# SJTU-IPADS/cocytus

Hardware: AMD Instinct MI355X
Metric: GiB/s device-resident RS(3,2) encode+decode, 4 KiB values (higher is better)
Workload: dtype u8

## Files before the change

cocytus_amd/csrc/cec_kernels.hpp:

```cpp
#pragma once

#include <hip/hip_runtime.h>
#include <stdint.h>

#include "gf256.hpp"

namespace cec {

constexpr int kTile = 4096;
constexpr int kBlock = 256;
constexpr int kBlockLog2 = 8;
constexpr uint64_t kLineBytes = 128;
static_assert(kBlock == 1 << kBlockLog2, "kBlock must be a power of two");
constexpr int kMaxStreams = 48;
constexpr int kPatN = 16;
constexpr int kPatL = 4;

enum : int32_t { kModeWrite = 0, kModeXor = 1 };

struct alignas(16) Pattern {
    int32_t n_in;
    int32_t n_out;
    int32_t in_stream[kPatN];
    int32_t in_src[kPatN];
// ... 283 lines not shown
                if (i < n_in) x[i] = ld16(in[i], pos);
#pragma unroll
            for (int l = 0; l < LT; ++l) {
                acc[l] = make_uint4(0, 0, 0, 0);
                if (l < n_out && is_acc(l)) acc[l] = ld16(out[l], pos);
            }
        } else {
#pragma unroll
            for (int i = 0; i < NT; ++i)
                if (i < n_in) x[i] = gather16(in[i], pos, cnt);
#pragma unroll
            for (int l = 0; l < LT; ++l) {
                acc[l] = make_uint4(0, 0, 0, 0);
                if (l < n_out && is_acc(l)) acc[l] = gather16(out[l], pos, cnt);
            }
        }
        if constexpr (Eng::kStaged) {
            const uint32_t nb = static_cast<uint32_t>(P->lds_rows) * 256u;
            if (nb) {
                const uint4 *src = reinterpret_cast<const uint4 *>(a.rows) + P->lds_row_base * 16;
                for (uint32_t b = threadIdx.x; b < nb / 16; b += blockDim.x) cec_lds_rows[b] = src[b];
                __syncthreads();
            }
            if (!active) continue;
        }
        compute_chunk<NT, LT, Eng>(P, n_in, n_out, x, acc, lds);
        if (wide) {
            bool wt = false;
            if constexpr (!Eng::kStaged) {
                wt = (a.flags & kFlagWriteThrough) != 0;
                if constexpr (S > kNarrowStreams) wt = wt || g >= a.wt_from;
            }
            if (wt) {
#pragma unroll
                for (int l = 0; l < LT; ++l)
                    if (l < n_out) st16_wt(out[l], pos, acc[l]);
            } else {
#pragma unroll
                for (int l = 0; l < LT; ++l)
                    if (l < n_out) st16(out[l], pos, acc[l]);
            }
        } else {
#pragma unroll
            for (int l = 0; l < LT; ++l)
                if (l < n_out) scatter16(out[l], pos, cnt, acc[l]);
        }
    }
    if constexpr (kSysRel) {
        __builtin_amdgcn_fence(__ATOMIC_RELEASE, "");
        __asm__ volatile("s_waitcnt vmcnt(0)" ::: "memory");
    }
}

constexpr int kScrubStreams = 24;

struct ScrubArgs {
    const uint8_t *base[kScrubStreams];
    const Tile *tiles;
    const Pattern *pattern;
    uint32_t *words;
    uint32_t *counter;
    uint64_t implicit_len;
    uint32_t n_tiles;
    uint32_t split_shift;
    uint32_t grid;
    uint32_t syn_shift;
};

template <int NT, int LT, bool kExact>
__global__ __launch_bounds__(kBlock) void scrub_kernel(ScrubArgs a) {
    const uint32_t sh = a.split_shift;
    const uint32_t g = blockIdx.x;
    if (g >= a.grid) return;
    const uint32_t t = g >> sh;
    const uint32_t part = g & ((1u << sh) - 1u);
    const uint32_t lane = (part << (kBlockLog2 - sh)) + threadIdx.x;
    const TileRef tr = load_tile(a, t);
    const CEC_CONST Pattern *P = as_const(a.pattern);
    const int n_in = kExact ? NT : P->n_in;
    const int n_out = kExact ? LT : P->n_out;

    const uint8_t *in[NT];
    const uint8_t *par[LT];
    uint64_t mis = 0;
#pragma unroll
    for (int i = 0; i < NT; ++i) {
        in[i] = nullptr;
        if (i < n_in) {
            in[i] = a.base[i] + tr.off;
            mis |= reinterpret_cast<uint64_t>(in[i]);
        }
    }
#pragma unroll
    for (int l = 0; l < LT; ++l) {
        par[l] = nullptr;
        if (l < n_out) {
            par[l] = a.base[n_in + l] + tr.off;
            mis |= reinterpret_cast<uint64_t>(par[l]);
        }
    }

    const uint32_t pos = lane * 16;
    if (pos >= tr.len) return;
    const uint32_t cnt = min(16u, tr.len - pos);
    uint4 x[NT];
    uint4 acc[LT];
// ... 317 lines not shown
```

cocytus_amd/csrc/cec_runtime.hip:

```cpp
#include <hip/hip_runtime.h>

#include <algorithm>
#include <atomic>
#include <chrono>
#include <cerrno>
#include <cstdarg>
#include <cstdio>
#include <cstdlib>
#include <cstring>
#include <map>
#include <mutex>
#include <string>
#include <vector>

#include "../../include/cocytus_ec.h"
#include "../../include/galois.h"
#include "../../include/jerasure.h"
#include "../../include/reed_sol.h"
#include "cec_hostplan.hpp"
#include "cec_kernels.hpp"
#include "cec_poolbook.hpp"
#include "gf256.hpp"

#define CEC_API extern "C" __attribute__((visibility("default")))
// ... 112 lines not shown

template <int NT, int LT, class Eng, int kAcc, bool kExact, int S = kMaxStreams, bool kSysRel = false>
static void launch_k(const CombineArgsN<S> &a, int grid, size_t lds, hipStream_t s) {
    hipLaunchKernelGGL((combine_kernel<NT, LT, Eng, kAcc, kExact, S, kSysRel>), dim3(grid),
                       dim3(kBlock >> a.split_shift), lds, s, a);
}

static CombineArgsN<kNarrowStreams> narrow_args(const CombineArgs &w) {
    CombineArgsN<kNarrowStreams> a;
    memset(&a, 0, sizeof a);
    for (int i = 0; i < kNarrowStreams; ++i) a.base[i] = w.base[i];
    a.tiles = w.tiles;
    a.patterns = w.patterns;
    a.rows = w.rows;
    a.implicit_len = w.implicit_len;
    a.n_tiles = w.n_tiles;
    a.split_shift = w.split_shift;
    a.grid = w.grid;
    a.flags = w.flags;
    return a;
}

template <class Eng>
static bool launch_narrow(int acc, const CombineArgsN<kNarrowStreams> &a, int grid, size_t lds, hipStream_t s) {
    const bool rel = (a.flags & kFlagSysRelease) != 0;
    if (acc == kAccAll && rel) launch_k<1, 1, Eng, kAccAll, true, kNarrowStreams, true>(a, grid, lds, s);
    else if (acc == kAccAll) launch_k<1, 1, Eng, kAccAll, true, kNarrowStreams>(a, grid, lds, s);
    else if (acc == kAccNone && rel) launch_k<1, 1, Eng, kAccNone, true, kNarrowStreams, true>(a, grid, lds, s);
    else if (acc == kAccNone) launch_k<1, 1, Eng, kAccNone, true, kNarrowStreams>(a, grid, lds, s);
    else return false;
    return true;
}

#define CEC_EXACT_WRITES(X, N) X(N, 1, kAccNone) X(N, 2, kAccNone) X(N, 3, kAccNone) X(N, 4, kAccNone)
#define CEC_EXACT_SHAPES(X)                                                                      \
    CEC_EXACT_WRITES(X, 1) CEC_EXACT_WRITES(X, 2) CEC_EXACT_WRITES(X, 3) CEC_EXACT_WRITES(X, 4)  \
    CEC_EXACT_WRITES(X, 5) CEC_EXACT_WRITES(X, 6) CEC_EXACT_WRITES(X, 7) CEC_EXACT_WRITES(X, 8)  \
    X(1, 1, kAccAll) X(2, 1, kAccAll) X(2, 2, kAccAll) X(2, 3, kAccAll) X(2, 4, kAccAll)         \
    X(2, 2, kAccAllButLast) X(2, 3, kAccAllButLast) X(2, 4, kAccAllButLast)

template <class Eng>
static bool launch_exact(int n, int l, int acc, const CombineArgs &a, int grid, size_t lds,
                         hipStream_t s) {
#define CEC_X(N, L, A)                                           \
    if (n == N && l == L && acc == A) {                          \
        launch_k<N, L, Eng, A, true>(a, grid, lds, s);       \
        return true;                                             \
    }
    CEC_EXACT_SHAPES(CEC_X)
#undef CEC_X
    return false;
}

static bool has_exact(int n, int l, int acc) {
#define CEC_X(N, L, A) if (n == N && l == L && acc == A) return true;
    CEC_EXACT_SHAPES(CEC_X)
#undef CEC_X
    return false;
}

struct Capacity {
    int nt, lt;
};
#define CEC_LT_RUNGS(lt, NT, K)                  \
    if (lt <= 1) { K(NT, 1) }                    \
    else if (lt <= 2) { K(NT, 2) }               \
    else { K(NT, 4) }
#define CEC_CAPACITY_RUNGS_FROM_4(nt, lt, K)     \
    if (nt <= 4) { CEC_LT_RUNGS(lt, 4, K) }      \
    else if (nt <= 8) { CEC_LT_RUNGS(lt, 8, K) } \
    else { CEC_LT_RUNGS(lt, 16, K) }
#define CEC_CAPACITY_RUNGS(nt, lt, K)            \
    if (nt <= 2) { CEC_LT_RUNGS(lt, 2, K) }      \
    else { CEC_CAPACITY_RUNGS_FROM_4(nt, lt, K) }

template <class Eng>
static Capacity launch_generic(int nt, int lt, const CombineArgs &a, int grid, size_t lds, hipStream_t s) {
#define CEC_G(NT, LT)                                              \
    launch_k<NT, LT, Eng, kAccRuntime, false>(a, grid, lds, s);   \
    return {NT, LT};
    CEC_CAPACITY_RUNGS(nt, lt, CEC_G)
#undef CEC_G
}

static bool exact_shape(const std::vector<Pattern> &pats, const std::vector<char> *used, int *n, int *l,
                        int *acc) {
    const Pattern *p0 = nullptr;
    for (size_t i = 0; i < pats.size(); ++i) {
        if (used && !(*used)[i]) continue;
        const Pattern &p = pats[i];
        if (!p0) {
            p0 = &p;
            continue;
        }
        if (p.n_in != p0->n_in || p.n_out != p0->n_out) return false;
        for (int o = 0; o < p.n_out; ++o)
            if (p.out_mode[o] != p0->out_mode[o]) return false;
    }
    if (!p0) return false;
    int nx = 0;
    for (int o = 0; o < p0->n_out; ++o) nx += p0->out_mode[o] == kModeXor;
    if (nx == 0) *acc = kAccNone;
    else if (nx == p0->n_out) *acc = kAccAll;
    else if (nx == p0->n_out - 1 && p0->out_mode[p0->n_out - 1] == kModeWrite) *acc = kAccAllButLast;
    else return false;
    *n = p0->n_in;
    *l = p0->n_out;
    return true;
}

#include "cec_combo.inc"

static inline size_t tiles_of(uint64_t off, uint32_t len) {
    return len ? static_cast<size_t>((off % kTile + len + kTile - 1) / kTile) : 0;
}
static inline size_t append_tiles(Tile *t, uint64_t off, uint64_t src_off, uint32_t len,
                                  uint32_t pattern) {
    size_t n = 0;
    for (uint32_t o = 0; o < len;) {
        const uint32_t phase = static_cast<uint32_t>((off + o) % kTile);
        const uint32_t step = std::min<uint32_t>(kTile - phase, len - o);
        t[n++] = Tile{off + o, src_off + o, step, pattern};
        o += step;
    }
    return n;
}
static inline int64_t count_line_tiles(const Tile *t, size_t n) {
    int64_t c = 0;
    for (size_t i = 0; i < n; ++i) c += t[i].len == kTile && (t[i].off & (kLineBytes - 1)) == 0;
    return c;
}

struct cec_plan {
    int device = -1;
    int n_ext = 0;
    int64_t n_tiles = 0;
    uint64_t total = 0;
    bool overlap = false;
    int64_t n_line_tiles = 0;
    Tile *d_tiles = nullptr;
    uint32_t max_pattern = 0;
    uint64_t max_end = 0;
    int max_end_ext = -1;
    std::vector<Tile> h_tiles;
    mutable Tracker uses;
};

CEC_API int cec_plan_destroy(cec_plan *p) {
    if (!p) return CEC_OK;
    int rc = CEC_OK;
    if (hipError_t e = p->uses.wait(p->device); e != hipSuccess)
        rc = fail(CEC_EHIP, "cec_plan_destroy: a launch of this plan failed: %s", hipGetErrorString(e));
    dev_cache().release(p->device, p->d_tiles, sizeof(Tile) * p->n_tiles);
    delete p;
    return rc;
}

CEC_API int cec_plan_release_stream(cec_plan *p, void *stream) {
    if (!p) return fail(CEC_EINVAL, "cec_plan_release_stream: plan is NULL");
    if (hipError_t e = p->uses.release(p->device, static_cast<hipStream_t>(stream)); e != hipSuccess)
        return fail(CEC_EHIP, "cec_plan_release_stream: %s", hipGetErrorString(e));
    return CEC_OK;
}
CEC_API int cec_plan_tracked_streams(const cec_plan *p) { return p ? static_cast<int>(p->uses.size()) : 0; }

CEC_API int cec_plan_create(cec_plan **out, const cec_extent *ext, int n, void *stream) {
    if (!out || n < 0 || (n > 0 && !ext)) return fail(CEC_EINVAL, "cec_plan_create: bad args");
    *out = nullptr;
    int dev;
    if (int r = current_device(&dev)) return r;
    cec_plan *p = new (std::nothrow) cec_plan;
    if (!p) return fail(CEC_ENOMEM, "cec_plan_create: host allocation");
    p->device = dev;
    p->n_ext = n;
    for (int e = 0; e < n; ++e) {
        p->max_pattern = std::max(p->max_pattern, ext[e].pattern);
        if (!ext[e].len) continue;
        const uint64_t end = ext[e].off > UINT64_MAX - ext[e].len ? UINT64_MAX : ext[e].off + ext[e].len;
        if (p->max_end_ext < 0 || end > p->max_end) {
            p->max_end = end;
            p->max_end_ext = e;
        }
    }
    size_t total_tiles = 0;
    for (int e = 0; e < n; ++e) total_tiles += tiles_of(ext[e].off, ext[e].len);
    p->h_tiles.resize(total_tiles);
    size_t nt = 0;
    for (int e = 0; e < n; ++e) {
        p->total += ext[e].len;
        nt += append_tiles(p->h_tiles.data() + nt, ext[e].off, ext[e].src_off, ext[e].len, ext[e].pattern);
    }
    if (p->h_tiles.size() > 0xFFFFFFFFull) {
        delete p;
        return fail(CEC_EINVAL, "cec_plan_create: more than 2^32 tiles");
    }
    p->n_tiles = static_cast<int64_t>(p->h_tiles.size());
    p->n_line_tiles = count_line_tiles(p->h_tiles.data(), p->h_tiles.size());
    {
        std::vector<std::pair<uint64_t, uint64_t>> r;
        r.reserve(n);
        for (int e = 0; e < n; ++e)
            if (ext[e].len) r.emplace_back(ext[e].off, ext[e].off + ext[e].len);
        std::sort(r.begin(), r.end());
        for (size_t i = 1; i < r.size(); ++i)
            if (r[i].first < r[i - 1].second) { p->overlap = true; break; }
    }
    hipStream_t s = static_cast<hipStream_t>(stream);
    if (p->n_tiles > 0) {
        const size_t bytes = sizeof(Tile) * p->n_tiles;
        p->d_tiles = static_cast<Tile *>(dev_cache().acquire(dev, bytes));
        if (!p->d_tiles) {
            delete p;
            return fail(CEC_ENOMEM, "cec_plan_create: %zu bytes of tiles", bytes);
        }
        if (hipMemcpyAsync(p->d_tiles, p->h_tiles.data(), bytes, hipMemcpyHostToDevice, s) != hipSuccess) {
            (void)hipGetLastError();
            cec_plan_destroy(p);
            return fail(CEC_EHIP, "cec_plan_create: tile upload failed");
        }
        p->uses.note(s);
    }
    *out = p;
    return CEC_OK;
}

CEC_API int cec_plan_num_extents(const cec_plan *p) { return p ? p->n_ext : 0; }
CEC_API int64_t cec_plan_num_tiles(const cec_plan *p) { return p ? p->n_tiles : 0; }
CEC_API uint64_t cec_plan_total_bytes(const cec_plan *p) { return p ? p->total : 0; }

struct TileSource {
    const Tile *tiles = nullptr;
    uint64_t n_tiles = 0;
    uint64_t n_line_tiles = 0;
    uint64_t implicit_len = 0;
    Tracker *uses = nullptr;

    static int of_plan(const cec_plan *plan, int dev, TileSource *out) {
        if (plan->device != dev)
            return fail(CEC_EINVAL, "plan built on device %d used on device %d", plan->device, dev);
        *out = {plan->d_tiles, static_cast<uint64_t>(plan->n_tiles), static_cast<uint64_t>(plan->n_line_tiles), 0,
                &plan->uses};
        return CEC_OK;
    }
    static int of_region(uint64_t len, TileSource *out) {
        const uint64_t n = (len + kTile - 1) / kTile;
        if (n > 0xFFFFFFFFull) return fail(CEC_EINVAL, "region too large");
        *out = {nullptr, n, n, len, nullptr};
        return CEC_OK;
    }
    static TileSource window(const Tile *d, const Tile *h, size_t n) {
        return {d, n, static_cast<uint64_t>(count_line_tiles(h, n)), 0, nullptr};
    }
    static TileSource whole_units(const Tile *d, size_t n) { return {d, n, n, 0, nullptr}; }
};

struct WaveTiles {
    Tile *h;
    size_t n = 0;
    std::vector<size_t> first;
    int cur = -1;
    explicit WaveTiles(Tile *host) : h(host) {}
    void begin_wave() { first.push_back(n); }
    void enter(int wave) {
        if (wave != cur) begin_wave();
        cur = wave;
    }
    void add(uint64_t off, uint64_t src_off, uint32_t len, uint32_t pattern) {
        n += append_tiles(h + n, off, src_off, len, pattern);
    }
    int waves() const { return static_cast<int>(first.size()); }
    TileSource all(const Tile *d) const { return TileSource::window(d, h, n); }
    TileSource window(int w, const Tile *d) const {
        const size_t lo = first[w], hi = w + 1 < waves() ? first[w + 1] : n;
        return TileSource::window(d + lo, h + lo, hi - lo);
    }
};

static uint32_t split_shift_for(const Streams &st, const TileSource &src) {
    static const int forced = [] {
        const char *e = getenv("CEC_SPLIT_SHIFT");
        return e && *e ? std::min(2, std::max(0, atoi(e))) : -1;
    }();
    if (forced >= 0) return static_cast<uint32_t>(forced);
    uintptr_t mis = 0;
    for (int i = 0; i < kMaxStreams; ++i) mis |= reinterpret_cast<uintptr_t>(st.base[i]);
    const bool full = src.n_line_tiles * 4 >= src.n_tiles * 3;
    return full && (mis & (kLineBytes - 1)) == 0 ? 2u : 0u;
}

static std::atomic<int> g_waves_per_cu{[] {
    const char *e = getenv("CEC_WAVES_PER_CU");
    return e && *e ? std::max(0, atoi(e)) : 0;
}()};
static int waves_per_cu_cap() { return g_waves_per_cu.load(std::memory_order_relaxed); }

static size_t occupancy_lds(int dev, uint32_t split_shift) {
    const int cap = waves_per_cu_cap();
    if (cap <= 0) return 0;
    const int waves_per_wg = (kBlock >> split_shift) / 64;
    const int wgs = std::max(1, cap / std::max(1, waves_per_wg));
    const size_t per_cu = g_dev[dev].lds_per_cu;
    const size_t lds = per_cu / static_cast<size_t>(wgs);
    return std::min<size_t>(65536, lds > 256 ? lds - 256 : 0);
}

enum { kStoreAuto = 0, kStoreNt = 1, kStoreWt = 2 };
// ... 3 lines not shown
    if (!strcmp(e, "wt")) return static_cast<int>(kStoreWt);
    if (!strcmp(e, "nt")) return static_cast<int>(kStoreNt);
    fprintf(stderr, "libcocytus_ec: CEC_STORE_POLICY=%s is not nt, wt or auto; using auto\n", e);
    return static_cast<int>(kStoreAuto);
}();
static uint64_t parse_byte_count(const char *name, uint64_t dflt) {
    const char *e = getenv(name);
    if (!e || !*e) return dflt;
    char *end = nullptr;
    errno = 0;
    const unsigned long long v = (*e >= '0' && *e <= '9') ? strtoull(e, &end, 0) : 0;
    if (!(*e >= '0' && *e <= '9') || !end || *end || errno == ERANGE) {
        fprintf(stderr, "libcocytus_ec: %s=%s is not a byte count; using %llu\n", name, e,
                static_cast<unsigned long long>(dflt));
        return dflt;
    }
    return static_cast<uint64_t>(v);
}
static const uint64_t g_wt_max_bytes = parse_byte_count("CEC_WT_MAX_BYTES", uint64_t(512) << 20);
CEC_API int cec_internal_store_policy(uint64_t *wt_max_bytes) {
    if (wt_max_bytes) *wt_max_bytes = g_wt_max_bytes;
    return g_store_policy;
}
static const uint64_t g_wt_tail_bytes = parse_byte_count("CEC_WT_TAIL_BYTES", uint64_t(96) << 20);

struct StoreChoice {
    bool all;
    uint64_t from;
};
static StoreChoice write_through(uint64_t n_tiles, uint32_t split_shift, int lt, uint64_t streamed) {
    if (g_store_policy != kStoreAuto) return {g_store_policy == kStoreWt, kNoWtTail};
    if (streamed <= g_wt_max_bytes) return {true, kNoWtTail};
    if (g_wt_tail_bytes == 0 || lt <= 0) return {false, kNoWtTail};
    const uint64_t per_item = static_cast<uint64_t>(lt) * (kTile >> split_shift);
    const uint64_t items = g_wt_tail_bytes / per_item + (g_wt_tail_bytes % per_item != 0);
    const uint64_t n_work = n_tiles << split_shift;
    if (items >= n_work) return {true, kNoWtTail};
    return {false, n_work - items};
}
CEC_API int cec_internal_wt_from(uint64_t n_tiles, uint32_t split_shift, int lt, uint64_t streamed,
                                 uint64_t *wt_tail_bytes, uint64_t *wt_from) {
    if (split_shift > 2 || n_tiles > 0xFFFFFFFFull) return fail(CEC_EINVAL, "cec_internal_wt_from: bad args");
    const StoreChoice c = write_through(n_tiles, split_shift, lt, streamed);
    if (wt_tail_bytes) *wt_tail_bytes = g_wt_tail_bytes;
    if (wt_from) *wt_from = c.from;
    return c.all ? 2 : c.from != kNoWtTail ? 1 : 0;
}

struct LaunchShape {
    int nt = 1, lt = 0, max_rows = 0;
    bool exact = false;
    int en = 0, el = 0, eacc = 0;
    int streams = 0;
};

static LaunchShape launch_shape(const std::vector<Pattern> &pats, const std::vector<char> *used) {
    LaunchShape sh;
    for (size_t i = 0; i < pats.size(); ++i) {
        if (used && !(*used)[i]) continue;
        sh.nt = std::max(sh.nt, pats[i].n_in);
        sh.lt = std::max(sh.lt, pats[i].n_out);
        sh.max_rows = std::max(sh.max_rows, pats[i].lds_rows);
        for (int j = 0; j < pats[i].n_in; ++j) sh.streams = std::max(sh.streams, pats[i].in_stream[j] + 1);
        for (int j = 0; j < pats[i].n_out; ++j) sh.streams = std::max(sh.streams, pats[i].out_stream[j] + 1);
    }
    sh.exact = exact_shape(pats, used, &sh.en, &sh.el, &sh.eacc);
    return sh;
}

enum KernelKind { kKindNarrow, kKindExact, kKindGeneric };
static_assert(kKindNarrow == CEC_KERNEL_NARROW && kKindExact == CEC_KERNEL_EXACT &&
                  kKindGeneric == CEC_KERNEL_GENERIC, "cec_launch_record::kind");
static_assert(kAccNone == CEC_ACC_NONE && kAccAll == CEC_ACC_ALL && kAccAllButLast == CEC_ACC_ALL_BUT_LAST &&
                  kAccRuntime == CEC_ACC_RUNTIME, "cec_launch_record::acc");
static_assert(kFlagSysRelease == CEC_LAUNCH_SYS_RELEASE && kFlagWriteThrough == CEC_LAUNCH_WRITE_THROUGH &&
                  kFlagWtTail == CEC_LAUNCH_WT_TAIL, "cec_launch_record::flags");

static thread_local cec_launch_record t_last_launch = {0, -1, 0, 0, -1, -1, 0, 0, 0, 0, 0, kNoWtTail};

static void record_launch(int kind, Capacity cap, int acc, bool lds, uint32_t split_shift, uint32_t flags,
                          uint32_t grid, uint64_t n_tiles, size_t lds_bytes, uint64_t wt_from = kNoWtTail) {
    t_last_launch = {t_last_launch.seq + 1, kind, cap.nt, cap.lt, acc, lds ? CEC_ENGINE_LDS : CEC_ENGINE_PERM,
                     split_shift, flags, grid, n_tiles, lds_bytes, wt_from};
}

CEC_API int cec_last_launch(cec_launch_record *out) {
    if (!out) return fail(CEC_EINVAL, "cec_last_launch: out is NULL");
    *out = t_last_launch;
    return CEC_OK;
}

static thread_local int t_fail_after = -1;
CEC_API int cec_internal_fail_launch(int after) {
    t_fail_after = after < 0 ? -1 : after;
    return CEC_OK;
}
static int launch_countdown() {
    if (t_fail_after == 0) {
        t_fail_after = -1;
        return fail(CEC_EHIP, "injected launch failure (cec_internal_fail_launch)");
    }
    if (t_fail_after > 0) --t_fail_after;
    return CEC_OK;
}

static int pattern_tables(int dev, const std::vector<Pattern> &pats, const std::vector<uint8_t> &rows,
                          hipStream_t s, PatEntry **entry) {
    std::string key(reinterpret_cast<const char *>(pats.data()), pats.size() * sizeof(Pattern));
    key.append(reinterpret_cast<const char *>(rows.data()), rows.size());
    return pattern_get(dev, std::move(key), s, entry);
}

struct Tables {
    const uint8_t *d;
    size_t n_pats;
    const Pattern *host;
    const std::vector<char> *used;
};

static bool stream_layout_ok(const uint8_t *const *bases, int slots, const Tables &tb) {
    for (size_t q = 0; q < tb.n_pats; ++q) {
        if (tb.used && (q >= tb.used->size() || !(*tb.used)[q])) continue;
        const Pattern &p = tb.host[q];
        for (int i = 0; i < p.n_in; ++i)
            if (p.in_stream[i] >= slots || !bases[p.in_stream[i]]) return false;
        for (int l = 0; l < p.n_out; ++l)
            if (p.out_stream[l] >= slots || !bases[p.out_stream[l]]) return false;
    }
    return true;
}

static bool layout_ok_for(const CombineArgs &a, const CombineArgsN<kNarrowStreams> *narrow, const Tables &tb) {
    return narrow ? stream_layout_ok(narrow->base, kNarrowStreams, tb) : stream_layout_ok(a.base, kMaxStreams, tb);
}

static int launch_combine(int dev, const Streams &st, const Tables &tb, const LaunchShape &sh, bool lds,
                          const TileSource &src, hipStream_t stream, uint32_t flags = 0, bool *released = nullptr) {
    if (st.refused) return fail(CEC_EINVAL, "internal: an op names more than %d byte streams; not launched", kMaxStreams);
    CombineArgs a;
    memset(&a, 0, sizeof a);
    a.flags = flags;
    const bool exact_k = sh.exact && has_exact(sh.en, sh.el, sh.eacc);
    const KernelKind kind =
        exact_k && sh.en == 1 && sh.el == 1 && sh.streams <= kNarrowStreams &&
                (sh.eacc == kAccAll || sh.eacc == kAccNone)
            ? kKindNarrow
            : exact_k ? kKindExact : kKindGeneric;
    for (int i = 0; i < kMaxStreams; ++i) a.base[i] = st.base[i];
    a.tiles = src.tiles;
    a.implicit_len = src.implicit_len;
    a.patterns = reinterpret_cast<const Pattern *>(tb.d);
    a.rows = tb.d + tb.n_pats * sizeof(Pattern);
    a.n_tiles = static_cast<uint32_t>(src.n_tiles);
    a.split_shift = split_shift_for(st, src);
    const StoreChoice wt = write_through(src.n_tiles, a.split_shift, sh.lt,
                                         src.n_tiles * kTile * static_cast<uint64_t>(sh.nt + sh.lt));
    a.wt_from = kind == kKindNarrow || lds ? kNoWtTail : wt.from;
    a.flags |= (wt.all ? kFlagWriteThrough : 0u) | (a.wt_from != kNoWtTail ? kFlagWtTail : 0u);
    const size_t lds_bytes = std::max(lds ? static_cast<size_t>(sh.max_rows) * 256 : 0,
                                      occupancy_lds(dev, a.split_shift));
    const uint64_t max_wgs = 0xFFFFFFFFull / (kBlock >> a.split_shift);
    const int grid = static_cast<int>(std::min<uint64_t>(src.n_tiles << a.split_shift, max_wgs));
    a.grid = static_cast<uint32_t>(grid);
    CombineArgsN<kNarrowStreams> na;
    if (kind == kKindNarrow) na = narrow_args(a);
    if (!layout_ok_for(a, kind == kKindNarrow ? &na : nullptr, tb))
        return fail(CEC_EINVAL, "internal: a launch's argument block cannot serve its patterns "
                                "(kind %d, %d x %d); not launched", static_cast<int>(kind), sh.en, sh.el);
    bool ok;
    Capacity cap = {sh.en, sh.el};
    if (kind == kKindNarrow) {
        ok = lds ? launch_narrow<LdsEngine>(sh.eacc, na, grid, lds_bytes, stream)
                 : launch_narrow<PermEngine>(sh.eacc, na, grid, lds_bytes, stream);
    } else if (kind == kKindExact) {
        ok = lds ? launch_exact<LdsEngine>(sh.en, sh.el, sh.eacc, a, grid, lds_bytes, stream)
                 : launch_exact<PermEngine>(sh.en, sh.el, sh.eacc, a, grid, lds_bytes, stream);
    } else {
        cap = lds ? launch_generic<LdsEngine>(sh.nt, sh.lt, a, grid, lds_bytes, stream)
                  : launch_generic<PermEngine>(sh.nt, sh.lt, a, grid, lds_bytes, stream);
        ok = true;
    }
    if (!ok) return fail(CEC_EINVAL, "internal: no %s kernel for %d x %d", kind == kKindNarrow ? "narrow" : "exact",
                         sh.en, sh.el);
    if (released) *released = kind == kKindNarrow && (flags & kFlagSysRelease) != 0;
    record_launch(kind, cap, kind == kKindGeneric ? static_cast<int>(kAccRuntime) : sh.eacc, lds, a.split_shift,
                  a.flags, a.grid, src.n_tiles, lds_bytes, a.wt_from);
    return CEC_OK;
}

static int run_combine(int dev, const Streams &st, const std::vector<Pattern> &pats,
                       const std::vector<uint8_t> &rows, const TileSource &src, hipStream_t stream,
                       const std::vector<char> *used, int engine) {
    if (int r = launch_countdown()) return r;
    if (src.n_tiles == 0 || pats.empty()) return CEC_OK;
    const LaunchShape sh = launch_shape(pats, used);
    if (sh.lt == 0) return CEC_OK;
    PatEntry *entry = nullptr;
    if (int r = pattern_tables(dev, pats, rows, stream, &entry)) return r;
    const int rc = launch_combine(dev, st, Tables{entry->d, pats.size(), pats.data(), used}, sh,
                                  engine == CEC_ENGINE_LDS, src, stream);
    if (src.uses) src.uses->note(stream);
    pattern_done(entry);
    if (rc) return rc;
    HIP_TRY(hipGetLastError());
    return CEC_OK;
}

static int build_patterns(const std::vector<Combo> &combos, size_t g, int engine, std::vector<Pattern> &pats,
                          std::vector<uint8_t> &rows, bool only_group = false) {
    for (const Combo &c : combos) {
        if (c.n_in < 0 || c.n_in > kPatN)
            return fail(CEC_EINVAL, "internal: a combination of %d inputs (a pattern holds %d); not launched",
                        c.n_in, kPatN);
        if (only_group && c.outs.size() > (g + 1) * kPatL)
            return fail(CEC_EINVAL, "internal: a combination of %zu outputs in one launch (a pattern holds %d); "
                                    "not launched", c.outs.size(), kPatL);
    }
    pats.reserve(pats.size() + combos.size());
    for (const Combo &c : combos) {
        Pattern p = blank_pattern();
        p.n_in = c.n_in;
        for (int i = 0; i < c.n_in; ++i) {
            p.in_stream[i] = c.in_stream[i];
            p.in_src[i] = c.in_src[i];
        }
        const size_t n = c.outs.size();
        const size_t lo = g * kPatL, hi = std::min(n, lo + kPatL);
        int no = 0;
        for (size_t o = lo; o < hi; ++o, ++no) {
            const Combo::Out &q = c.outs[o];
            p.out_stream[no] = q.stream;
            p.out_src[no] = q.src;
            p.out_mode[no] = q.mode;
            for (int i = 0; i < c.n_in; ++i) set_coef(p, no, i, q.coef[i], engine);
        }
        p.n_out = no;
        if (engine == CEC_ENGINE_LDS) assign_rows(p, rows);
        pats.push_back(p);
    }
    return CEC_OK;
}

static int run_combos(int dev, const Streams &st, const std::vector<Combo> &combos, const TileSource &src,
                      hipStream_t stream, const std::vector<char> *used = nullptr, bool lds_op = false) {
    size_t max_out = 0;
    for (const Combo &c : combos) max_out = std::max(max_out, c.outs.size());
    const int engine = op_engine(lds_op);
    const size_t groups = (max_out + kPatL - 1) / kPatL;
    for (size_t g = 0; g < groups; ++g) {
        std::vector<Pattern> pats;
        std::vector<uint8_t> rows;
        if (int r = build_patterns(combos, g, engine, pats, rows)) return r;
// ... 735 lines not shown
```

cocytus_amd/ec.py:

```python
from __future__ import annotations

import ctypes
import os
from typing import Iterable, Sequence

HERE = os.path.dirname(os.path.abspath(__file__))
LIB_PATH = os.environ.get("CEC_LIB_PATH") or os.path.join(HERE, "libcocytus_ec.so")

CEC_OK = 0
CEC_EINVAL = -1
CEC_ESINGULAR = -2
CEC_EHIP = -3
CEC_ENOMEM = -4
CEC_EOVERLAP = -5
CEC_ENODEV = -6
CEC_EFULL = -7
CEC_ENGINE_PERM = 0
CEC_ENGINE_LDS = 1
CEC_ENGINE_AUTO = 2
CEC_MAX_K = 16
CEC_MAX_M = 8
UNIT_SIZE = 4096

_STATUS = {
# ... 33 lines not shown


class RegionJob(ctypes.Structure):

    _fields_ = [
        ("src", ctypes.c_void_p),
        ("dst", ctypes.c_void_p),
        ("base", ctypes.c_void_p),
        ("len", ctypes.c_uint32),
        ("multby", ctypes.c_int32),
        ("add", ctypes.c_int32),
    ]


class BatchStats(ctypes.Structure):
    _fields_ = [("launches", ctypes.c_int), ("rounds", ctypes.c_int), ("plan_us", ctypes.c_float),
                ("pack_us", ctypes.c_float), ("gpu_us", ctypes.c_float), ("unpack_us", ctypes.c_float),
                ("in_place_launches", ctypes.c_int)]


class CacheInfo(ctypes.Structure):

    _fields_ = [(n, ctypes.c_uint64) for n in (
        "pattern_entries", "pattern_bytes", "pattern_uploads", "pattern_evictions",
        "pattern_entry_limit", "device_cached_bytes", "pinned_cached_bytes")]


class SyncRecord(ctypes.Structure):
    _fields_ = [("seq", ctypes.c_uint64), ("host_results", ctypes.c_int),
                ("waves_released", ctypes.c_int), ("fenced", ctypes.c_int)]


class LaunchRecord(ctypes.Structure):
    _fields_ = [("seq", ctypes.c_uint64), ("kind", ctypes.c_int), ("nt", ctypes.c_int),
                ("lt", ctypes.c_int), ("acc", ctypes.c_int), ("engine", ctypes.c_int),
                ("split_shift", ctypes.c_uint32), ("flags", ctypes.c_uint32), ("grid", ctypes.c_uint32),
                ("n_tiles", ctypes.c_uint64), ("lds_bytes", ctypes.c_uint64), ("wt_from", ctypes.c_uint64)]


CEC_KERNEL_NARROW, CEC_KERNEL_EXACT, CEC_KERNEL_GENERIC = 0, 1, 2
CEC_KERNEL_SCRUB = 3
CEC_KERNEL_DIGEST = 4
CEC_KERNEL_DIGEST_CHECK = 5
CEC_KERNEL_DIGEST_UPDATE = 6
DIGEST_BYTES = 32
CEC_SCRUB_UNLOCATED = -1


class ScrubFinding(ctypes.Structure):
    _fields_ = [("tile", ctypes.c_uint64), ("off", ctypes.c_uint64), ("len", ctypes.c_uint32),
                ("syndromes", ctypes.c_uint32), ("ruled_out", ctypes.c_uint32), ("lid", ctypes.c_int32)]

CEC_ACC_NONE, CEC_ACC_ALL, CEC_ACC_ALL_BUT_LAST, CEC_ACC_RUNTIME = 0, 1, 2, 3
CEC_LAUNCH_SYS_RELEASE, CEC_LAUNCH_WRITE_THROUGH, CEC_LAUNCH_WT_TAIL = 1, 2, 4
CEC_NO_WT_TAIL = 2**64 - 1

_vp = ctypes.c_void_p
_i = ctypes.c_int
_u32 = ctypes.c_uint32
_ip = ctypes.POINTER(ctypes.c_int)
_pp = ctypes.POINTER(ctypes.c_void_p)

_SIGS = {
    "cec_version": ([], ctypes.c_char_p),
    "cec_last_error": ([], ctypes.c_char_p),
    "cec_device_check": ([], _i),
    "cec_set_engine": ([_i], _i),
    "cec_get_engine": ([], _i),
    "cec_last_engine": ([], _i),
    "cec_internal_check_launch_layout": ([_i, _ip, _i, _ip, _i, _pp, _i], _i),
    "cec_internal_store_policy": ([ctypes.POINTER(ctypes.c_uint64)], _i),
    "cec_internal_wt_from": ([ctypes.c_uint64, _u32, _i, ctypes.c_uint64, ctypes.POINTER(ctypes.c_uint64),
                              ctypes.POINTER(ctypes.c_uint64)], _i),
    "cec_internal_fail_launch": ([_i], _i),
    "cec_plan_release_stream": ([_vp, _vp], _i),
    "cec_plan_tracked_streams": ([_vp], _i),
    "cec_drainer_release_stream": ([_vp, _vp], _i),
    "cec_recovery_release_stream": ([_vp, _vp], _i),
    "cec_recovery_pool_release_stream": ([_vp, _vp], _i),
    "cec_set_waves_per_cu": ([_i], _i),
    "cec_get_waves_per_cu": ([], _i),
    "cec_plan_create": ([ctypes.POINTER(_vp), ctypes.POINTER(Extent), _i, _vp], _i),
    "cec_plan_destroy": ([_vp], _i),
    "cec_plan_num_extents": ([_vp], _i),
    "cec_plan_num_tiles": ([_vp], ctypes.c_int64),
    "cec_plan_total_bytes": ([_vp], ctypes.c_uint64),
    "cec_region_multiply": ([_vp, _i, ctypes.c_size_t, _vp, _i, _vp], _i),
    "cec_encode": ([_i, _i, _ip, _pp, _pp, _vp, _vp], _i),
    "cec_encode_region": ([_i, _i, _ip, _pp, _pp, ctypes.c_size_t, _vp], _i),
    "cec_diff_update": ([_i, _i, _ip, _pp, _vp, _pp, _i, _vp, _vp], _i),
    "cec_set_diff": ([_i, _pp, _vp, _vp, _vp, _vp], _i),
    "cec_apply_diffs": ([_i, _i, _ip, _i, _vp, _vp, _vp, _vp], _i),
    "cec_residual": ([_i, _i, _ip, _i, _u32, _pp, _vp, _vp, _vp], _i),
    "cec_solve": ([_i, _i, _ip, _u32, _pp, _pp, _vp, _vp], _i),
    "cec_decode": ([_i, _i, _ip, ctypes.POINTER(_u32), _i, _pp, _pp, _vp, _vp], _i),
    "cec_recovery_mask": ([_i, _i, _i, _ip], _u32),
    "cec_arena_stride": ([ctypes.c_size_t], ctypes.c_size_t),
    "cec_arenas_alloc": ([_i, ctypes.c_size_t, _pp, ctypes.POINTER(_vp)], _i),
    "cec_arenas_free": ([_vp], _i),
    "cec_drainer_create": ([ctypes.POINTER(_vp), _i, _i, _ip, _i, ctypes.c_size_t], _i),
    "cec_drainer_destroy": ([_vp], _i),
    "cec_drainer_apply": ([_vp, ctypes.POINTER(HostUpdate), _i, _vp, _vp], _i),
    "cec_drainer_last_launches": ([_vp], _i),
    "cec_drainer_validate": ([_vp, ctypes.POINTER(HostUpdate), _i], _i),
    "cec_region_multiply_batch": ([ctypes.POINTER(RegionJob), _i, _vp], _i),
    "cec_region_multiply_batch_stats": ([ctypes.POINTER(BatchStats)], _i),
    "cec_drainer_staging": ([_vp, ctypes.POINTER(ctypes.c_size_t)], ctypes.POINTER(ctypes.c_uint8)),
# ... 865 lines not shown
```

include/cocytus_ec.h:

```cpp
#ifndef COCYTUS_EC_H
#define COCYTUS_EC_H

#include <stddef.h>
#include <stdint.h>

#ifdef __cplusplus
extern "C" {
#endif

#define CEC_MAX_K 16
#define CEC_MAX_M 8
#define CEC_UNIT_SIZE 4096

typedef enum cec_status {
    CEC_OK = 0,
    CEC_EINVAL = -1,
    CEC_ESINGULAR = -2,
    CEC_EHIP = -3,
    CEC_ENOMEM = -4,
    CEC_EOVERLAP = -5,
    CEC_ENODEV = -6,
    CEC_EFULL = -7
} cec_status;

// ... 184 lines not shown
                     const uint8_t *const *parity, size_t len, void *stream);
int64_t cec_scrub_wait(cec_scrub_report *s);
int cec_scrub_findings(cec_scrub_report *s, cec_scrub_finding *out, int cap);
int cec_scrub_classify(uint32_t word, int k, int m, const int *matrix);
int cec_scrub_repair(cec_scrub_report *s, int k, int m, const int *matrix, uint8_t *const *data,
                     uint8_t *const *parity, void *stream, int *unrepaired);

#define CEC_DIGEST_BYTES 32
int cec_digest(int n, const uint8_t *const *arenas, uint8_t *const *digests,
               const cec_plan *plan, void *stream);
int cec_digest_region(int n, const uint8_t *const *arenas, uint8_t *const *digests,
                      size_t len, void *stream);
int cec_scrub_digests(cec_scrub_report *s, int k, int m, const int *matrix,
                      const uint8_t *const *data_digests, const uint8_t *const *parity_digests,
                      const cec_plan *plan, void *stream);
int cec_scrub_digests_region(cec_scrub_report *s, int k, int m, const int *matrix,
                             const uint8_t *const *data_digests, const uint8_t *const *parity_digests,
                             size_t len, void *stream);

int cec_digest_apply_diffs(int k, int m, const int *matrix, int lid_self, const uint8_t *diffs,
                           uint8_t *digests, uint64_t n_units, const cec_plan *plan, void *stream);

int cec_digest_verify_region(cec_scrub_report *s, const uint8_t *live, const uint8_t *fresh,
                             size_t len, void *stream);

typedef struct cec_cache_info {
    uint64_t pattern_entries;
    uint64_t pattern_bytes;
    uint64_t pattern_uploads;
    uint64_t pattern_evictions;
    uint64_t pattern_entry_limit;
    uint64_t device_cached_bytes;
    uint64_t pinned_cached_bytes;
} cec_cache_info;
int cec_cache_get_info(cec_cache_info *out);
int cec_cache_set_pattern_limit(int entries);
int cec_cache_trim(void);

typedef struct cec_sync_record {
    uint64_t seq;
    int host_results;
    int waves_released;
    int fenced;
} cec_sync_record;
int cec_last_sync(cec_sync_record *out);

enum { CEC_KERNEL_NARROW = 0, CEC_KERNEL_EXACT = 1, CEC_KERNEL_GENERIC = 2,
       CEC_KERNEL_SCRUB = 3 ,
       CEC_KERNEL_DIGEST = 4 ,
       CEC_KERNEL_DIGEST_CHECK = 5 ,
       CEC_KERNEL_DIGEST_UPDATE = 6  };
enum { CEC_ACC_NONE = 0, CEC_ACC_ALL = 1, CEC_ACC_ALL_BUT_LAST = 2, CEC_ACC_RUNTIME = 3 };
enum { CEC_LAUNCH_SYS_RELEASE = 1, CEC_LAUNCH_WRITE_THROUGH = 2,
       CEC_LAUNCH_WT_TAIL = 4  };
#define CEC_NO_WT_TAIL UINT64_MAX
typedef struct cec_launch_record {
    uint64_t seq;
    int kind;
    int nt, lt;
    int acc;
    int engine;
    uint32_t split_shift;
    uint32_t flags;
    uint32_t grid;
    uint64_t n_tiles;
    uint64_t lds_bytes;
    uint64_t wt_from;
} cec_launch_record;
int cec_last_launch(cec_launch_record *out);

int cec_internal_check_launch_layout(int narrow, const int *in_slots, int n_in, const int *out_slots,
                                     int n_out, const void *const *bases, int n_bases);
int cec_internal_store_policy(uint64_t *wt_max_bytes);
int cec_internal_wt_from(uint64_t n_tiles, uint32_t split_shift, int lt, uint64_t streamed,
                         uint64_t *wt_tail_bytes, uint64_t *wt_from);
int cec_internal_fail_launch(int after);

int cec_event_create(void **ev);
int cec_event_destroy(void *ev);
int cec_event_record(void *ev, void *stream);
int cec_event_elapsed_ms(void *start, void *stop, float *ms);
int cec_stream_synchronize(void *stream);
int cec_device_count(int *count);
int cec_set_device(int device);
int cec_stream_create(void **stream);
int cec_stream_destroy(void *stream);
int cec_copy(void *dst, const void *src, size_t n, void *stream);
int cec_host_register(void *p, size_t bytes, uint8_t **device_alias);
int cec_host_unregister(void *p);

#ifdef __cplusplus
}
#endif
#endif
```

Baseline: 2692.

## Add specialized whole-tile exact kernel with packed per-pattern scalar records

Adds a whole_tile_kernel for exact shapes when every tile is a full, 16-byte-aligned 4 KiB unit. It reads a compact per-pattern record (slot bytes, src bits, coefficient classes, multiply tables) into scalar registers, skips zero and identity coefficients, and drops the bounds and scatter handling of the generic exact kernel. The goal is less per-workgroup setup and fewer scalar loads in the small RS(3,2) encode/decode launches. The records are uploaded alongside the pattern tables and take part in the cache key, and the path can be turned off with an environment variable.

```diff
diff --git a/cocytus_amd/csrc/cec_kernels.hpp b/cocytus_amd/csrc/cec_kernels.hpp
--- a/cocytus_amd/csrc/cec_kernels.hpp
+++ b/cocytus_amd/csrc/cec_kernels.hpp
@@ -359,6 +359,151 @@
     }
 }
 
+constexpr uint32_t kFlagWholeTile = 8u;
+constexpr int kWholeMaxIn = 8;
+constexpr int kWholePreloadTabs = 8;
+
+struct WholeHead {
+    uint32_t in_slot[kWholeMaxIn / 4];
+    uint32_t out_slot;
+    uint32_t src;
+    uint32_t cls[2];
+    uint32_t pad[2];
+};
+static_assert(sizeof(WholeHead) == 32, "one s_load_dwordx8");
+template <int NT, int LT>
+struct alignas(32) WholeRec {
+    WholeHead head;
+    uint32_t tab[LT * NT][5];
+};
+static_assert(kPatL * kWholeMaxIn * 2 <= 64, "WholeHead::cls");
+constexpr uint32_t whole_rec_stride(int nt, int lt) {
+    return (static_cast<uint32_t>(sizeof(WholeHead)) + 20u * nt * lt + 31u) & ~31u;
+}
+
+struct WholeArgs {
+    uint8_t *base[kMaxStreams];
+    const Tile *tiles;
+    const uint8_t *recs;
+    uint32_t wt_from;
+    uint32_t split_shift;
+    uint32_t flags;
+    uint32_t pad;
+};
+
+template <int NT, int LT, int kAcc>
+__global__ __launch_bounds__(kBlock) void whole_tile_kernel(WholeArgs a) {
+    static_assert(NT <= kWholeMaxIn && LT <= kPatL && kAcc != kAccRuntime, "exact shapes only");
+    using Rec = WholeRec<NT, LT>;
+    static_assert(sizeof(Rec) == whole_rec_stride(NT, LT), "record stride");
+    constexpr bool kPreload = NT * LT <= kWholePreloadTabs;
+    uint32_t sh = a.split_shift, flags = a.flags, wt_from = a.wt_from;
+    uint64_t tiles = reinterpret_cast<uint64_t>(a.tiles), recs = reinterpret_cast<uint64_t>(a.recs);
+    __asm__ volatile("" : "+s"(sh), "+s"(flags), "+s"(wt_from), "+s"(tiles), "+s"(recs));
+    const uint32_t g = blockIdx.x;
+    const uint32_t t = g >> sh;
+    const uint32_t part = g & ((1u << sh) - 1u);
+    const uint32_t pos = ((part << (kBlockLog2 - sh)) + threadIdx.x) * 16;
+    uint64_t off = static_cast<uint64_t>(t) * kTile, src_off = off;
+    uint32_t pat = 0;
+    if (tiles != 0) {
+        const CEC_CONST Tile *tl = reinterpret_cast<const CEC_CONST Tile *>(tiles) + t;
+        off = tl->off;
+        src_off = tl->src_off;
+        pat = tl->pattern;
+    }
+    const CEC_CONST Rec *R = (const CEC_CONST Rec *)(recs + static_cast<uint64_t>(pat) * sizeof(Rec));
+    WholeHead h;
+    h.in_slot[0] = R->head.in_slot[0];
+    h.in_slot[1] = R->head.in_slot[1];
+    h.out_slot = R->head.out_slot;
+    h.src = R->head.src;
+    h.cls[0] = R->head.cls[0];
+    h.cls[1] = R->head.cls[1];
+    uint64_t base[NT + LT];
+#pragma unroll
+    for (int i = 0; i < NT; ++i)
+        base[i] = reinterpret_cast<uint64_t>(a.base[(h.in_slot[i >> 2] >> (8 * (i & 3))) & 0xFFu]);
+#pragma unroll
+    for (int l = 0; l < LT; ++l) base[NT + l] = reinterpret_cast<uint64_t>(a.base[(h.out_slot >> (8 * l)) & 0xFFu]);
+    uint32_t wt = (flags & kFlagWriteThrough) | static_cast<uint32_t>((static_cast<uint64_t>(wt_from) - g - 1u) >> 63);
+    __builtin_amdgcn_sched_barrier(0);
+    const uint8_t *in[NT];
+    uint8_t *out[LT];
+#pragma unroll
+    for (int i = 0; i < NT; ++i)
+        in[i] = reinterpret_cast<const uint8_t *>(base[i] + ((h.src >> i) & 1u ? src_off : off));
+    uint64_t *ob = base + NT;
+    if constexpr (LT == 1) __asm__ volatile("" : "+s"(wt), "+s"(ob[0]));
+    else if constexpr (LT == 2) __asm__ volatile("" : "+s"(wt), "+s"(ob[0]), "+s"(ob[1]));
+    else if constexpr (LT == 3) __asm__ volatile("" : "+s"(wt), "+s"(ob[0]), "+s"(ob[1]), "+s"(ob[2]));
+    else __asm__ volatile("" : "+s"(wt), "+s"(ob[0]), "+s"(ob[1]), "+s"(ob[2]), "+s"(ob[3]));
+#pragma unroll
+    for (int l = 0; l < LT; ++l)
+        out[l] = reinterpret_cast<uint8_t *>(ob[l] + ((h.src >> (8 + l)) & 1u ? src_off : off));
+
+    uint4 x[NT];
+    uint4 acc[LT];
+#pragma unroll
+    for (int i = 0; i < NT; ++i) x[i] = ld16(in[i], pos);
+#pragma unroll
+    for (int l = 0; l < LT; ++l) {
+        const bool rmw = kAcc == kAccAll || (kAcc == kAccAllButLast && l < LT - 1);
+        acc[l] = rmw ? ld16(out[l], pos) : make_uint4(0, 0, 0, 0);
+    }
+    __builtin_amdgcn_sched_barrier(0);
+    uint32_t tab[kPreload ? LT * NT : 1][5];
+    if constexpr (kPreload) {
+#pragma unroll
+        for (int q = 0; q < LT * NT; ++q)
+#pragma unroll
+            for (int w = 0; w < 5; ++w) tab[q][w] = R->tab[q][w];
+        __builtin_amdgcn_sched_barrier(0);
+#pragma unroll
+        for (int q = 0; q < LT * NT; ++q)
+            __asm__ volatile("" : "+s"(tab[q][0]), "+s"(tab[q][1]), "+s"(tab[q][2]), "+s"(tab[q][3]), "+s"(tab[q][4]));
+    }
+#pragma unroll
+    for (int i = 0; i < NT; ++i) {
+        const uint32_t xv[4] = {x[i].x, x[i].y, x[i].z, x[i].w};
+        PermEngine::Sel s[4];
+#pragma unroll
+        for (int w = 0; w < 4; ++w) s[w] = PermEngine::sel(xv[w]);
+#pragma unroll
+        for (int l = 0; l < LT; ++l) {
+            constexpr int kPerWord = 16;
+            const int q = l * NT + i;
+            const uint32_t c = (h.cls[q / kPerWord] >> (2 * (q % kPerWord))) & 3u;
+            if (c == 0) continue;
+            uint32_t p[4];
+            if (c == 1) {
+#pragma unroll
+                for (int w = 0; w < 4; ++w) p[w] = xv[w];
+            } else if constexpr (kPreload) {
+#pragma unroll
+                for (int w = 0; w < 4; ++w)
+                    p[w] = __builtin_amdgcn_perm(tab[q][1], tab[q][0], s[w].s0) ^
+                           __builtin_amdgcn_perm(tab[q][3], tab[q][2], s[w].s1) ^
+                           __builtin_amdgcn_perm(tab[q][4], tab[q][4], s[w].s2);
+            } else {
+#pragma unroll
+                for (int w = 0; w < 4; ++w) p[w] = PermEngine::mul(s[w], R->tab[q], nullptr);
+            }
+            acc[l].x ^= p[0];
+            acc[l].y ^= p[1];
+            acc[l].z ^= p[2];
+            acc[l].w ^= p[3];
+        }
+    }
+    if (wt) {
+#pragma unroll
+        for (int l = 0; l < LT; ++l) st16_wt(out[l], pos, acc[l]);
+    } else {
+#pragma unroll
+        for (int l = 0; l < LT; ++l) st16(out[l], pos, acc[l]);
+    }
+}
+
 constexpr int kScrubStreams = 24;
 
 struct ScrubArgs {
diff --git a/cocytus_amd/csrc/cec_runtime.hip b/cocytus_amd/csrc/cec_runtime.hip
--- a/cocytus_amd/csrc/cec_runtime.hip
+++ b/cocytus_amd/csrc/cec_runtime.hip
@@ -188,6 +188,17 @@
     return false;
 }
 
+static bool launch_whole(int n, int l, int acc, const WholeArgs &a, int grid, size_t lds, hipStream_t s) {
+#define CEC_X(N, L, A)                                                                        \
+    if (n == N && l == L && acc == A) {                                                       \
+        hipLaunchKernelGGL((whole_tile_kernel<N, L, A>), dim3(grid), dim3(kBlock >> a.split_shift), lds, s, a); \
+        return true;                                                                          \
+    }
+    CEC_EXACT_SHAPES(CEC_X)
+#undef CEC_X
+    return false;
+}
+
 static bool has_exact(int n, int l, int acc) {
 #define CEC_X(N, L, A) if (n == N && l == L && acc == A) return true;
     CEC_EXACT_SHAPES(CEC_X)
@@ -266,6 +277,18 @@
     for (size_t i = 0; i < n; ++i) c += t[i].len == kTile && (t[i].off & (kLineBytes - 1)) == 0;
     return c;
 }
+struct WholeCount {
+    uint64_t off = 0, src = 0;
+};
+static inline WholeCount count_whole_tiles(const Tile *t, size_t n) {
+    WholeCount c;
+    for (size_t i = 0; i < n; ++i) {
+        const bool w = t[i].len == kTile && (t[i].off & 15) == 0;
+        c.off += w;
+        c.src += w && (t[i].src_off & 15) == 0;
+    }
+    return c;
+}
 
 struct cec_plan {
     int device = -1;
@@ -274,6 +297,7 @@
     uint64_t total = 0;
     bool overlap = false;
     int64_t n_line_tiles = 0;
+    WholeCount whole;
     Tile *d_tiles = nullptr;
     uint32_t max_pattern = 0;
     uint64_t max_end = 0;
@@ -332,6 +356,7 @@
     }
     p->n_tiles = static_cast<int64_t>(p->h_tiles.size());
     p->n_line_tiles = count_line_tiles(p->h_tiles.data(), p->h_tiles.size());
+    p->whole = count_whole_tiles(p->h_tiles.data(), p->h_tiles.size());
     {
         std::vector<std::pair<uint64_t, uint64_t>> r;
         r.reserve(n);
@@ -370,24 +395,26 @@
     uint64_t n_line_tiles = 0;
     uint64_t implicit_len = 0;
     Tracker *uses = nullptr;
+    WholeCount whole = {};
 
     static int of_plan(const cec_plan *plan, int dev, TileSource *out) {
         if (plan->device != dev)
             return fail(CEC_EINVAL, "plan built on device %d used on device %d", plan->device, dev);
         *out = {plan->d_tiles, static_cast<uint64_t>(plan->n_tiles), static_cast<uint64_t>(plan->n_line_tiles), 0,
-                &plan->uses};
+                &plan->uses, plan->whole};
         return CEC_OK;
     }
     static int of_region(uint64_t len, TileSource *out) {
         const uint64_t n = (len + kTile - 1) / kTile;
         if (n > 0xFFFFFFFFull) return fail(CEC_EINVAL, "region too large");
-        *out = {nullptr, n, n, len, nullptr};
+        const uint64_t whole = len / kTile;
+        *out = {nullptr, n, n, len, nullptr, {whole, whole}};
         return CEC_OK;
     }
     static TileSource window(const Tile *d, const Tile *h, size_t n) {
-        return {d, n, static_cast<uint64_t>(count_line_tiles(h, n)), 0, nullptr};
-    }
-    static TileSource whole_units(const Tile *d, size_t n) { return {d, n, n, 0, nullptr}; }
+        return {d, n, static_cast<uint64_t>(count_line_tiles(h, n)), 0, nullptr, count_whole_tiles(h, n)};
+    }
+    static TileSource whole_units(const Tile *d, size_t n) { return {d, n, n, 0, nullptr, {}}; }
 };
 
 struct WaveTiles {
@@ -497,6 +524,7 @@
     bool exact = false;
     int en = 0, el = 0, eacc = 0;
     int streams = 0;
+    bool by_src = false;
 };
 
 static LaunchShape launch_shape(const std::vector<Pattern> &pats, const std::vector<char> *used) {
@@ -506,8 +534,14 @@
         sh.nt = std::max(sh.nt, pats[i].n_in);
         sh.lt = std::max(sh.lt, pats[i].n_out);
         sh.max_rows = std::max(sh.max_rows, pats[i].lds_rows);
-        for (int j = 0; j < pats[i].n_in; ++j) sh.streams = std::max(sh.streams, pats[i].in_stream[j] + 1);
-        for (int j = 0; j < pats[i].n_out; ++j) sh.streams = std::max(sh.streams, pats[i].out_stream[j] + 1);
+        for (int j = 0; j < pats[i].n_in; ++j) {
+            sh.streams = std::max(sh.streams, pats[i].in_stream[j] + 1);
+            sh.by_src = sh.by_src || pats[i].in_src[j] != 0;
+        }
+        for (int j = 0; j < pats[i].n_out; ++j) {
+            sh.streams = std::max(sh.streams, pats[i].out_stream[j] + 1);
+            sh.by_src = sh.by_src || pats[i].out_src[j] != 0;
+        }
     }
     sh.exact = exact_shape(pats, used, &sh.en, &sh.el, &sh.eacc);
     return sh;
@@ -519,7 +553,8 @@
 static_assert(kAccNone == CEC_ACC_NONE && kAccAll == CEC_ACC_ALL && kAccAllButLast == CEC_ACC_ALL_BUT_LAST &&
                   kAccRuntime == CEC_ACC_RUNTIME, "cec_launch_record::acc");
 static_assert(kFlagSysRelease == CEC_LAUNCH_SYS_RELEASE && kFlagWriteThrough == CEC_LAUNCH_WRITE_THROUGH &&
-                  kFlagWtTail == CEC_LAUNCH_WT_TAIL, "cec_launch_record::flags");
+                  kFlagWtTail == CEC_LAUNCH_WT_TAIL && kFlagWholeTile == CEC_LAUNCH_WHOLE_TILE,
+              "cec_launch_record::flags");
 
 static thread_local cec_launch_record t_last_launch = {0, -1, 0, 0, -1, -1, 0, 0, 0, 0, 0, kNoWtTail};
 
@@ -550,10 +585,43 @@
 }
 
 static int pattern_tables(int dev, const std::vector<Pattern> &pats, const std::vector<uint8_t> &rows,
-                          hipStream_t s, PatEntry **entry) {
+                          hipStream_t s, PatEntry **entry, const std::vector<uint8_t> &recs = {}) {
     std::string key(reinterpret_cast<const char *>(pats.data()), pats.size() * sizeof(Pattern));
     key.append(reinterpret_cast<const char *>(rows.data()), rows.size());
+    key.append(reinterpret_cast<const char *>(recs.data()), recs.size());
     return pattern_get(dev, std::move(key), s, entry);
+}
+
+static const bool g_whole_tile = [] {
+    const char *e = getenv("CEC_WHOLE_TILE");
+    return !(e && *e && atoi(e) == 0);
+}();
+
+static std::vector<uint8_t> whole_records(const std::vector<Pattern> &pats, int n, int l) {
+    const size_t stride = whole_rec_stride(n, l);
+    std::vector<uint8_t> recs(pats.size() * stride, 0);
+    for (size_t q = 0; q < pats.size(); ++q) {
+        const Pattern &p = pats[q];
+        if (p.n_in != n || p.n_out != l) continue;
+        WholeHead h;
+        memset(&h, 0, sizeof h);
+        for (int i = 0; i < n; ++i) {
+            h.in_slot[i >> 2] |= static_cast<uint32_t>(p.in_stream[i] & 0xFF) << (8 * (i & 3));
+            h.src |= static_cast<uint32_t>(p.in_src[i] != 0) << i;
+        }
+        uint32_t *tab = reinterpret_cast<uint32_t *>(recs.data() + q * stride + sizeof h);
+        for (int o = 0; o < l; ++o) {
+            h.out_slot |= static_cast<uint32_t>(p.out_stream[o] & 0xFF) << (8 * o);
+            h.src |= static_cast<uint32_t>(p.out_src[o] != 0) << (8 + o);
+            for (int i = 0; i < n; ++i) {
+                const int at = o * n + i, c = p.coef[o][i];
+                h.cls[at / 16] |= static_cast<uint32_t>(c == 0 ? 0 : c == 1 ? 1 : 2) << (2 * (at % 16));
+                memcpy(tab + 5 * at, p.tab[o][i], 5 * sizeof(uint32_t));
+            }
+        }
+        memcpy(recs.data() + q * stride, &h, sizeof h);
+    }
+    return recs;
 }
 
 struct Tables {
@@ -561,6 +629,7 @@
     size_t n_pats;
     const Pattern *host;
     const std::vector<char> *used;
+    const uint8_t *recs = nullptr;
 };
 
 static bool stream_layout_ok(const uint8_t *const *bases, int slots, const Tables &tb) {
@@ -604,6 +673,18 @@
     a.flags |= (wt.all ? kFlagWriteThrough : 0u) | (a.wt_from != kNoWtTail ? kFlagWtTail : 0u);
     const size_t lds_bytes = std::max(lds ? static_cast<size_t>(sh.max_rows) * 256 : 0,
                                       occupancy_lds(dev, a.split_shift));
+    bool whole = g_whole_tile && kind == kKindExact && !lds && tb.recs &&
+                 src.n_tiles <= (0xFFFFFFFFull / kBlock) &&
+                 (sh.by_src ? src.whole.src : src.whole.off) == src.n_tiles;
+    for (size_t q = 0; whole && q < tb.n_pats; ++q) {
+        if (tb.used && (q >= tb.used->size() || !(*tb.used)[q])) continue;
+        const Pattern &p = tb.host[q];
+        uintptr_t mis = 0;
+        for (int i = 0; i < p.n_in; ++i) mis |= reinterpret_cast<uintptr_t>(st.base[p.in_stream[i]]);
+        for (int l = 0; l < p.n_out; ++l) mis |= reinterpret_cast<uintptr_t>(st.base[p.out_stream[l]]);
+        whole = (mis & 15) == 0;
+    }
+    if (whole) a.flags |= kFlagWholeTile;
     const uint64_t max_wgs = 0xFFFFFFFFull / (kBlock >> a.split_shift);
     const int grid = static_cast<int>(std::min<uint64_t>(src.n_tiles << a.split_shift, max_wgs));
     a.grid = static_cast<uint32_t>(grid);
@@ -617,6 +698,16 @@
     if (kind == kKindNarrow) {
         ok = lds ? launch_narrow<LdsEngine>(sh.eacc, na, grid, lds_bytes, stream)
                  : launch_narrow<PermEngine>(sh.eacc, na, grid, lds_bytes, stream);
+    } else if (whole) {
+        WholeArgs w;
+        memset(&w, 0, sizeof w);
+        for (int i = 0; i < kMaxStreams; ++i) w.base[i] = a.base[i];
+        w.tiles = a.tiles;
+        w.recs = tb.recs;
+        w.wt_from = static_cast<uint32_t>(std::min<uint64_t>(a.wt_from, 0xFFFFFFFFull));
+        w.split_shift = a.split_shift;
+        w.flags = a.flags;
+        ok = launch_whole(sh.en, sh.el, sh.eacc, w, grid, lds_bytes, stream);
     } else if (kind == kKindExact) {
         ok = lds ? launch_exact<LdsEngine>(sh.en, sh.el, sh.eacc, a, grid, lds_bytes, stream)
                  : launch_exact<PermEngine>(sh.en, sh.el, sh.eacc, a, grid, lds_bytes, stream);
@@ -641,8 +732,12 @@
     const LaunchShape sh = launch_shape(pats, used);
     if (sh.lt == 0) return CEC_OK;
     PatEntry *entry = nullptr;
-    if (int r = pattern_tables(dev, pats, rows, stream, &entry)) return r;
-    const int rc = launch_combine(dev, st, Tables{entry->d, pats.size(), pats.data(), used}, sh,
+    const bool with_recs = g_whole_tile && engine != CEC_ENGINE_LDS && sh.exact && has_exact(sh.en, sh.el, sh.eacc);
+    std::vector<uint8_t> recs;
+    if (with_recs) recs = whole_records(pats, sh.en, sh.el);
+    if (int r = pattern_tables(dev, pats, rows, stream, &entry, recs)) return r;
+    const uint8_t *d_recs = with_recs ? entry->d + pats.size() * sizeof(Pattern) + rows.size() : nullptr;
+    const int rc = launch_combine(dev, st, Tables{entry->d, pats.size(), pats.data(), used, d_recs}, sh,
                                   engine == CEC_ENGINE_LDS, src, stream);
     if (src.uses) src.uses->note(stream);
     pattern_done(entry);
diff --git a/cocytus_amd/ec.py b/cocytus_amd/ec.py
--- a/cocytus_amd/ec.py
+++ b/cocytus_amd/ec.py
@@ -109,7 +109,7 @@
                 ("syndromes", ctypes.c_uint32), ("ruled_out", ctypes.c_uint32), ("lid", ctypes.c_int32)]
 
 CEC_ACC_NONE, CEC_ACC_ALL, CEC_ACC_ALL_BUT_LAST, CEC_ACC_RUNTIME = 0, 1, 2, 3
-CEC_LAUNCH_SYS_RELEASE, CEC_LAUNCH_WRITE_THROUGH, CEC_LAUNCH_WT_TAIL = 1, 2, 4
+CEC_LAUNCH_SYS_RELEASE, CEC_LAUNCH_WRITE_THROUGH, CEC_LAUNCH_WT_TAIL, CEC_LAUNCH_WHOLE_TILE = 1, 2, 4, 8
 CEC_NO_WT_TAIL = 2**64 - 1
 
 _vp = ctypes.c_void_p
diff --git a/include/cocytus_ec.h b/include/cocytus_ec.h
--- a/include/cocytus_ec.h
+++ b/include/cocytus_ec.h
@@ -260,7 +260,8 @@
        CEC_KERNEL_DIGEST_UPDATE = 6  };
 enum { CEC_ACC_NONE = 0, CEC_ACC_ALL = 1, CEC_ACC_ALL_BUT_LAST = 2, CEC_ACC_RUNTIME = 3 };
 enum { CEC_LAUNCH_SYS_RELEASE = 1, CEC_LAUNCH_WRITE_THROUGH = 2,
-       CEC_LAUNCH_WT_TAIL = 4  };
+       CEC_LAUNCH_WT_TAIL = 4 ,
+       CEC_LAUNCH_WHOLE_TILE = 8  };
 #define CEC_NO_WT_TAIL UINT64_MAX
 typedef struct cec_launch_record {
     uint64_t seq;
```

New measurement: 2697 (median of 6 runs). Within noise of the previous version (+0.2%).
